# Gadersd/whisper-burn

Hardware: NVIDIA H100
Metric: audio-seconds/sec (higher is better)
Workload: dtype f32 (fp16-exact weights, fp32 activations/accumulate)

## Files before the change

### whisper-burn_b200/csrc/decoder.h

```cpp
#pragma once
#include <stdint.h>

#include "../host/beam_fixed.hpp"
#include "wb_internal.h"

namespace wb {

constexpr int DEC_KC = 8;

struct DecLayer {
    const float *ln1_g, *ln1_b, *ln2_g, *ln2_b, *ln3_g, *ln3_b;
    float ln1_eps, ln2_eps, ln3_eps;
    const void *Wqkv, *Wo, *Wcq, *Wco, *W1, *W2;
    const float *bqkv, *bo, *bcq, *bco, *b1, *b2;
};
enum { D5_KIND_LN = 0, D5_KIND_ATTN, D5_KIND_GEMM };
enum { D5_ST_LN_EMB = 0, D5_ST_LN_FOLD, D5_ST_LN_FOLD_NOPUB, D5_ST_LN_X, D5_ST_PLANES, D5_ST_CROSS };
enum { D5_EM_QKV = 0, D5_EM_RESID, D5_EM_CQ, D5_EM_HID, D5_EM_PART, D5_EM_LOGITS };
struct Dec5Desc {
    int kind = D5_KIND_ATTN;
    const void* W = nullptr;
    const float* bias = nullptr;
    int N = 0, n_slabs = 1, stage = 0, emit = 0;
    const float *g = nullptr, *b = nullptr;
// ... 16 lines not shown
    const void* E_tiled = nullptr;
    const float *lnf_g = nullptr, *lnf_b = nullptr;
    float lnf_eps = 1e-5f;
    float *x = nullptr, *q = nullptr, *att = nullptr, *hid = nullptr;
    float* ypart = nullptr;
    const Dec5Desc* d5 = nullptr;
    void *att_pl = nullptr, *hid_pl = nullptr;
    float* lgbuf = nullptr;
    int lg_slices = 1;
    void *kc = nullptr, *vc = nullptr;
    const void* ckv = nullptr;
    int kv_half = 0;
    int kv_row0 = 0;
    const int* row_window = nullptr;
    const int64_t* win_row_off = nullptr;
    const int* win_T = nullptr;
    const int* anc = nullptr;
    int n_splits = 1;
    float *part_o = nullptr, *part_m = nullptr, *part_l = nullptr;
    int* tokens = nullptr;
    const int* cur_tok = nullptr;
    int use_cur_tok = 0;
    int pos0 = 0, n_steps = 1, logits_from = 0;
    const uint8_t* is_special = nullptr;
    int mask_mode = 0;
    int k = 1, greedy = 0, eot = -1;
    int *lengths = nullptr, *finished = nullptr;
    int *topk_id = nullptr;
    float* topk_lp = nullptr;
    float* logits_out = nullptr;
    float *lg_m = nullptr, *lg_s = nullptr, *lg_v = nullptr;
    int* lg_i = nullptr;
    int *pos = nullptr, *n_unfinished = nullptr, *steps_done = nullptr;
    unsigned int* bar = nullptr;
    const void* d6_pack = nullptr;
    const float* d6_params = nullptr;
    unsigned long long* trace = nullptr;
    int trace_cap = 0;
    int beam = 0, n_win = 0, max_depth = 0;
    int* anc_alt = nullptr;
    int* slot_live = nullptr;
    beamfx::Head* bm_head = nullptr;
    int* bm_seq = nullptr;
    int* bm_cnt = nullptr;
    int* bm_win = nullptr;
    int* bm_out = nullptr;
    int* bm_out_len = nullptr;
};
void launch_dec3(const DecArgs& a, int n_ctas, bool w_half, cudaStream_t st);
bool launch_dec4(const DecArgs& a, bool w_half, cudaStream_t st);
struct Dec6Pack {
    DevBuf<uint8_t> pack;
    DevBuf<float> params;
};
bool launch_dec6(DecArgs a, const Model& m, Dec6Pack& pack, cudaStream_t st);
struct Dec5Tables {
    DevBuf<Dec5Desc> unsplit;
    DevBuf<Dec5Desc> split;
};
void dec5_build_tables(const Model& m, int n_sm, Dec5Tables& t);
int launch_dec5(const DecArgs& a, const Dec5Tables& t, int n_ctas, bool w_half, cudaStream_t st);
size_t dec5_plane_uint4(int d);

void launch_dec_anc_identity(int* anc, int R, int t_max, cudaStream_t st);
void launch_dec_reorder(const int* anc_old, int* anc_new, const int* parent, const int* pos_ptr, int R, int t_max,
                        cudaStream_t st);

}
```

### whisper-burn_b200/csrc/decoder6.cu

```cuda
#include <cooperative_groups.h>

#include <cstdlib>

#include "dec_common.cuh"
#include "wgmma.cuh"

namespace cg = cooperative_groups;

namespace wb {

namespace {

constexpr int NCW = 8;
constexpr int NPROD = 1;
constexpr int W_PROD = NCW;
constexpr int NTH6 = (NCW + NPROD) * 32;
constexpr int SLOT = 16384;
constexpr int NSLOT = 8;
constexpr int LG_NBUF = 2;
constexpr int BX_SLAB = 1024;

template <int D>
struct Geo {
    static constexpr int H = D / 64, CS = H, NS = 4 * D / CS, SEND = D + 4;
    static constexpr int pad128(int n) { return (n + 127) / 128 * 128; }
    static constexpr int OFF_QKV = 0, OFF_O = OFF_QKV + 192 * D * 2, OFF_CQ = OFF_O + D * 64 * 2, OFF_CO = OFF_CQ + 64 * D * 2,
                         OFF_W1 = OFF_CO + D * 64 * 2, OFF_W2 = OFF_W1 + NS * D * 2, PACK = OFF_W2 + D * NS * 2;
    static_assert(D % 128 == 0 && NS % 128 == 0, "only the 192- and 64-row segments end in a 64-row tile");
    static constexpr int P_LN1G = 0, P_LN1B = D, P_LN2G = 2 * D, P_LN2B = 3 * D, P_LN3G = 4 * D, P_LN3B = 5 * D, P_BO = 6 * D,
                         P_BCO = 7 * D, P_B2 = 8 * D, P_BQKV = 9 * D, P_BCQ = 9 * D + 192, P_B1 = 9 * D + 256, P_EPS = 9 * D + 256 + NS, PARAMS = 9 * D + 256 + NS + 4;
    static constexpr int KMAX = D > NS ? D : NS;
    static_assert(PARAMS % 4 == 0 && SEND % 4 == 0 && NS % 64 == 0 && D % 64 == 0, "layout");
};

__device__ __forceinline__ uint32_t s32(const void* p) { return (uint32_t)__cvta_generic_to_shared(p); }
__device__ __forceinline__ void mbar_init(uint64_t* bar, uint32_t count) { asm volatile("mbarrier.init.shared::cta.b64 [%0], %1;" ::"r"(s32(bar)), "r"(count)); }
__device__ __forceinline__ void mbar_expect_tx(uint64_t* bar, uint32_t bytes) {
    asm volatile("mbarrier.arrive.expect_tx.shared::cta.b64 _, [%0], %1;" ::"r"(s32(bar)), "r"(bytes) : "memory");
}
__device__ __forceinline__ void mbar_arrive(uint64_t* bar) { asm volatile("mbarrier.arrive.shared::cta.b64 _, [%0];" ::"r"(s32(bar)) : "memory"); }
__device__ long long g_watchdog = 20000000000LL;
__device__ __forceinline__ void mbar_wait(uint64_t* bar, uint32_t parity) {
    const long long WATCHDOG = g_watchdog;
    const uint32_t b = s32(bar);
    const long long t0 = clock64();
    for (;;) {
        uint32_t done;
        asm volatile("{\n.reg .pred p;\nmbarrier.try_wait.parity.shared::cta.b64 p, [%1], %2;\nselp.u32 %0, 1, 0, p;\n}" : "=r"(done) : "r"(b), "r"(parity) : "memory");
        if (done) return;
        if (clock64() - t0 > WATCHDOG) __trap();
    }
}
__device__ __forceinline__ void bulk_g2s(void* dst, const void* src, uint32_t bytes, uint64_t* bar) {
    asm volatile("cp.async.bulk.shared::cluster.global.mbarrier::complete_tx::bytes [%0], [%1], %2, [%3];" ::"r"(s32(dst)), "l"(src), "r"(bytes), "r"(s32(bar)) : "memory");
}
__device__ __forceinline__ void bulk_s2peer(void* dst_local, const void* src, uint32_t bytes, uint64_t* bar_local, uint32_t rank) {
    uint32_t rd, rb;
    asm volatile("mapa.shared::cluster.u32 %0, %1, %2;" : "=r"(rd) : "r"(s32(dst_local)), "r"(rank));
    asm volatile("mapa.shared::cluster.u32 %0, %1, %2;" : "=r"(rb) : "r"(s32(bar_local)), "r"(rank));
    asm volatile("cp.async.bulk.shared::cluster.shared::cta.mbarrier::complete_tx::bytes [%0], [%1], %2, [%3];" ::"r"(rd), "r"(s32(src)), "r"(bytes), "r"(rb) : "memory");
}
__device__ __forceinline__ void bar_consumers() { asm volatile("bar.sync 1, 256;" ::: "memory"); }
__device__ __forceinline__ void bar_all() { asm volatile("bar.sync 2, %0;" ::"n"(NTH6) : "memory"); }
__device__ __forceinline__ float group8_sum(float v) {
    v += __shfl_xor_sync(0xffffffffu, v, 1);
    v += __shfl_xor_sync(0xffffffffu, v, 2);
    v += __shfl_xor_sync(0xffffffffu, v, 4);
    return v;
}
__device__ __host__ __forceinline__ uint32_t sw128_off(int row, int k, int slab_bytes) {
    return (uint32_t)((k >> 6) * slab_bytes + row * 128 + ((((k & 63) >> 3) ^ (row & 7)) << 4) + (k & 7) * 2);
}

template <typename KVT>
__device__ __forceinline__ int hdim(int l8, int i) {
    if constexpr (sizeof(KVT) == 4) return (i < 4 ? 4 * l8 : 32 + 4 * l8) + (i & 3);
    else return 8 * l8 + i;
}
template <typename KVT>
// ... 159 lines not shown
                }
                o.out[row] = v;
            } else if (o.mode == EM_CQ) {
                o.out[row] = __fmul_rn(__fadd_rn(s, o.bias[row]), o.scale);
            } else {
                o.out[row] = gelu_erf(__fadd_rn(s, o.bias[row]));
            }
        }
    }
    c.tile += (uint32_t)n_tiles;
    c.n += (uint32_t)(n_tiles * n_slabs);
    bar_consumers();
    return c;
}

template <int D>
__device__ __noinline__ void ln6(const float* x_s, const float* g, const float* b, float eps, int eps_outside, uint8_t* bx) {
    const int tid = threadIdx.x, lane = tid & 31;
    float v[D / 32];
    float sum = 0.0f;
#pragma unroll
    for (int i = 0; i < D / 32; ++i) { v[i] = x_s[lane + 32 * i]; sum += v[i]; }
    sum = warp_sum(sum);
    const float mean = __fdiv_rn(sum, (float)D);
    float q = 0.0f;
#pragma unroll
    for (int i = 0; i < D / 32; ++i) { const float dv = __fsub_rn(v[i], mean); q = __fadd_rn(q, __fmul_rn(dv, dv)); }
    q = warp_sum(q);
    const float var = __fdiv_rn(q, (float)D);
    const float den = eps_outside ? __fadd_rn(__fsqrt_rn(var), eps) : __fsqrt_rn(__fadd_rn(var, eps));
#pragma unroll 1
    for (int c = tid; c < D; c += 256) bx_store(bx, c, __fadd_rn(__fmul_rn(__fdiv_rn(__fsub_rn(x_s[c], mean), den), g[c]), b[c]));
}

__device__ __noinline__ void attn_merge6(const float* wm, const float* wl, const float* wo, uint8_t* bx, float* rec) {
    const int tid = threadIdx.x;
    bar_consumers();
    if (tid < 64) {
        float M = -INFINITY;
#pragma unroll
        for (int w2 = 0; w2 < NCW; ++w2) M = fmaxf(M, wm[w2]);
        float Ls = 0.0f, o = 0.0f;
#pragma unroll
        for (int w2 = 0; w2 < NCW; ++w2) {
            const float sc = wm[w2] > -INFINITY ? expf(wm[w2] - M) : 0.0f;
            Ls += sc * wl[w2];
            o += sc * wo[w2 * 64 + tid];
        }
        bx_store(bx, tid, o);
        if (tid == 0) { rec[0] = M; rec[1] = Ls; }
    }
}

enum { MODE_SUM = 0, MODE_ATTN = 1 };

template <int D>
__device__ __noinline__ void combine6(const float* pr, uint64_t* bar, uint32_t parity, int mode, const float* bias, float* x_s, float* wsrc_s) {
    constexpr int CS = Geo<D>::CS, SEND = Geo<D>::SEND;
    const int tid = threadIdx.x;
    if (tid == 0) mbar_expect_tx(bar, CS * SEND * 4);
    mbar_wait(bar, parity);
    if (tid < CS) {
        const float* me = pr + tid * SEND + D;
        wsrc_s[tid] = mode == MODE_SUM ? 1.0f : me[0] > -INFINITY ? __fdiv_rn(1.0f, me[1]) : 0.0f;
    }
    bar_consumers();
#pragma unroll 1
    for (int c = tid; c < D; c += 256) {
        float acc = bias[c];
#pragma unroll 4
        for (int s = 0; s < CS; ++s) acc = fmaf(wsrc_s[s], pr[s * SEND + c], acc);
        x_s[c] = __fadd_rn(x_s[c], acc);
    }
    bar_consumers();
}

template <typename KVT, bool ANC>
__device__ __forceinline__ void self_attn6_body(const float* qkv_s, const KVT* kbase, const KVT* vbase, int ld, int p, const int* anc,
                                                int64_t row_ld, float* wm, float* wl, float* wo) {
    const int warp = threadIdx.x >> 5, lane = threadIdx.x & 31, rg = lane >> 3, l8 = lane & 7;
    float q[8];
#pragma unroll
    for (int i = 0; i < 8; ++i) q[i] = qkv_s[hdim<KVT>(l8, i)];
    Softmax8 A;
    A.init();
    float kf[4][8], vf[4][8];
    const int j0 = warp * 4 + rg;
#pragma unroll
    for (int u = 0; u < 4; ++u) {
        const int j = j0 + 32 * u;
        if (j < p) {
            const int64_t off = ANC ? (int64_t)__ldcg(anc + j) * row_ld + (int64_t)j * ld : (int64_t)j * ld;
            load_row8<KVT>(kbase + off, l8, 0, kf[u], false);
            load_row8<KVT>(vbase + off, l8, 0, vf[u], false);
        } else if (j == p) {
#pragma unroll
            for (int i = 0; i < 8; ++i) { kf[u][i] = qkv_s[64 + hdim<KVT>(l8, i)]; vf[u][i] = qkv_s[128 + hdim<KVT>(l8, i)]; }
        } else {
#pragma unroll
            for (int i = 0; i < 8; ++i) { kf[u][i] = 0.0f; vf[u][i] = 0.0f; }
        }
    }
#pragma unroll
    for (int u = 0; u < 4; ++u) {
        float s = 0.0f;
#pragma unroll
        for (int i = 0; i < 8; ++i) s = fmaf(q[i], kf[u][i], s);
        s = group8_sum(s);
        if (j0 + 32 * u <= p) A.add(s, vf[u]);
    }
    A.merge_xor(8);
    A.merge_xor(16);
    if (rg == 0) {
#pragma unroll
        for (int i = 0; i < 8; ++i) wo[warp * 64 + hdim<KVT>(l8, i)] = A.o[i];
        if (l8 == 0) { wm[warp] = A.m; wl[warp] = A.l; }
    }
}
template <typename KVT>
__device__ __noinline__ void self_attn6(const float* qkv_s, const KVT* kbase, const KVT* vbase, int ld, int p, float* wm, float* wl, float* wo) {
    self_attn6_body<KVT, false>(qkv_s, kbase, vbase, ld, p, nullptr, 0, wm, wl, wo);
}
template <typename KVT>
__device__ __noinline__ void self_attn6_anc(const float* qkv_s, const KVT* kbase, const KVT* vbase, int ld, int p, const int* anc, int64_t row_ld,
                                            float* wm, float* wl, float* wo) {
    self_attn6_body<KVT, true>(qkv_s, kbase, vbase, ld, p, anc, row_ld, wm, wl, wo);
}

__device__ __forceinline__ void cand_insert(float* lv, int* li, float v, int n) {
    if (!(v > lv[DEC_KC - 1] || (v == lv[DEC_KC - 1] && n < li[DEC_KC - 1]))) return;
    int k = DEC_KC - 1;
    for (; k > 0 && (v > lv[k - 1] || (v == lv[k - 1] && n < li[k - 1])); --k) { lv[k] = lv[k - 1]; li[k] = li[k - 1]; }
    lv[k] = v;
    li[k] = n;
}

template <typename KVT>
__device__ __noinline__ uint32_t cross_attn6(const Pipe P, uint32_t n, int* slot_cnt, const float* q2_s, int T, float* wm, float* wl, float* wo) {
    constexpr int ROWB = 128 * (int)sizeof(KVT), KPC = SLOT / ROWB;
    const int warp = threadIdx.x >> 5, lane = threadIdx.x & 31, rg = lane >> 3, l8 = lane & 7;
    float q[8];
#pragma unroll
    for (int i = 0; i < 8; ++i) q[i] = q2_s[hdim<KVT>(l8, i)];
    Softmax8 A;
    A.init();
#pragma unroll 1
    for (int k0 = 0; k0 < T; k0 += KPC) {
        const int nk = min(KPC, T - k0);
        const uint32_t slot = n % NSLOT;
        mbar_wait(P.full + slot, (n / NSLOT) & 1);
        const uint8_t* blk = P.ring + slot * SLOT;
#pragma unroll 2
        for (int kk = warp * 4 + rg; kk < nk; kk += 32) {
            const int par = (k0 + kk) & 1;
            const KVT* rowp = reinterpret_cast<const KVT*>(blk + (size_t)kk * ROWB);
            float kf[8], vf[8];
            load_row8<KVT>(rowp, l8, par, kf, true);
            load_row8<KVT>(rowp + 64, l8, par, vf, true);
            float s = 0.0f;
#pragma unroll
            for (int i = 0; i < 8; ++i) s = fmaf(q[i], kf[i], s);
            const unsigned int gm = 0xffu << (lane & 24);
            s += __shfl_xor_sync(gm, s, 1);
            s += __shfl_xor_sync(gm, s, 2);
            s += __shfl_xor_sync(gm, s, 4);
            A.add(s, vf);
        }
        __syncwarp();
        if (lane == 0 && atomicAdd(slot_cnt + slot, 1) == NCW - 1) {
            slot_cnt[slot] = 0;
            mbar_arrive(P.empty + slot);
        }
        ++n;
    }
    __syncwarp();
    A.merge_xor(8);
    A.merge_xor(16);
    if (rg == 0) {
#pragma unroll
        for (int i = 0; i < 8; ++i) wo[warp * 64 + hdim<KVT>(l8, i)] = A.o[i];
        if (l8 == 0) { wm[warp] = A.m; wl[warp] = A.l; }
    }
    return n;
}

constexpr int BM_LIVE = 24;
constexpr int BM_NX = 3 * BM_LIVE + 3 * NCW * beamfx::MAX_NODES;
__device__ __noinline__ void finish_beam(const DecArgs& a, int p, int depth, const int* anc_cur, uint8_t* scratch, const int* live, int* nx,
                                         int* ctl) {
    namespace fx = beamfx;
    const int tid = threadIdx.x, warp = tid >> 5, lane = tid & 31;
    const int R = a.R, B = a.beam, t_max = a.t_max, NW = a.n_win;
    int* nx_par = nx;
    int* nx_tok = nx_par + BM_LIVE;
    int* nx_live = nx_tok + BM_LIVE;
    int* pk_src = nx_live + BM_LIVE + warp * 3 * fx::MAX_NODES;
    int* pk_tok = pk_src + fx::MAX_NODES;
    int* pk_len = pk_tok + fx::MAX_NODES;
    constexpr int RINGW = NSLOT * SLOT / NCW;
    static_assert(160 * DEC_KC * 8 <= RINGW, "finisher candidate scratch");
    for (int r = warp; r < R; r += NCW) {
        if (!live[r]) continue;
        const int NP = gridDim.x;
        float rm[5], rs[5];
#pragma unroll
        for (int k = 0; k < 5; ++k) {
            const int c = min(lane + 32 * k, NP - 1);
// ... 108 lines not shown
            const int s = pk_src[i], tk = pk_tok[i], ln = pk_len[i] - (tk >= 0 ? 1 : 0);
            for (int j = lane; j < ln; j += 32) dst[i * t_max + j] = __ldcg(src + s * t_max + j);
            if (lane == 0 && tk >= 0) dst[i * t_max + ln] = tk;
        }
        __syncwarp();
    }
    bar_consumers();
    if (tid == 0) {
        int open = 0;
        for (int w = 0; w < NW; ++w) open += __ldcg(a.bm_win + 2 * w + 1) ? 0 : 1;
        ctl[2] = (depth + 1 >= a.max_depth || open == 0) ? 1 : 0;
        ctl[3] = open;
    }
    bar_consumers();
    if (ctl[2] == 0) {
        int* an = (depth & 1) ? const_cast<int*>(a.anc) : a.anc_alt;
        if (tid < R) {
            a.slot_live[tid] = nx_live[tid];
            if (nx_live[tid]) a.tokens[(int64_t)tid * t_max + p + 1] = nx_tok[tid];
        }
        const int P = p + 2;
        for (int q = tid; q < R * P; q += 256) {
            const int r = q / P, j = q % P;
            if (nx_live[r]) an[(int64_t)r * t_max + j] = j <= p ? __ldcg(anc_cur + (int64_t)nx_par[r] * t_max + j) : r;
        }
    } else {
        for (int w = warp; w < NW; w += NCW) {
            const int buf = __ldcg(a.bm_win + 2 * w);
            const fx::Head* hs = a.bm_head + ((size_t)buf * NW + w) * fx::MAX_NODES;
            int best = 0, len = 0;
            if (lane == 0) {
                const int n = __ldcg(a.bm_cnt + buf * NW + w);
                fx::Head hn[fx::MAX_NODES];
                for (int b = 0; b < n; ++b) { hn[b].log_prob = __ldcg(&hs[b].log_prob); hn[b].finished = __ldcg(&hs[b].finished); }
                best = max(fx::max_by_last(hn, n), 0);
                len = n > 0 ? __ldcg(&hs[best].len) : 0;
                a.bm_out_len[w] = len;
            }
            best = __shfl_sync(0xffffffffu, best, 0);
            len = __shfl_sync(0xffffffffu, len, 0);
            const int* s = a.bm_seq + (((size_t)buf * NW + w) * fx::MAX_NODES + best) * t_max;
            for (int j = lane; j < len; j += 32) a.bm_out[(int64_t)w * t_max + j] = __ldcg(s + j);
        }
        if (tid == 0) {
            *a.steps_done = depth + 1;
            *a.pos = p + 1;
            *a.n_unfinished = ctl[3];
            a.bar[3] = 1;
        }
    }
    bar_consumers();
}

template <int D, int NT8, typename KVT, bool BEAM = false>
__global__ void __launch_bounds__(NTH6, 1)
dec6_kernel(const DecArgs a) {
    using G = Geo<D>;
    constexpr int CS = G::CS, NS = G::NS, SEND = G::SEND, PARAMS = G::PARAMS;
    constexpr int KPC = SLOT / (128 * (int)sizeof(KVT));
    constexpr int ROWB = 128 * (int)sizeof(KVT);
    extern __shared__ __align__(1024) unsigned char smraw_[];
    uint8_t* smraw = reinterpret_cast<uint8_t*>((reinterpret_cast<uintptr_t>(smraw_) + 1023) & ~(uintptr_t)1023);
    cg::cluster_group cl = cg::this_cluster();
    const int tid = threadIdx.x, warp = tid >> 5, lane = tid & 31;
    const int rank = (int)cl.block_rank(), h = rank;
    const int cluster_id = blockIdx.x / CS, n_clusters = gridDim.x / CS;
    const int L = a.L, V = a.V, R = a.R, t_max = a.t_max;

    uint8_t* ring_mem = smraw;
    uint8_t* bx = ring_mem + NSLOT * SLOT;
    float* params = reinterpret_cast<float*>(bx + (G::KMAX / 64) * BX_SLAB);
    float* part = params + 2 * PARAMS;
    float* y_s = part + 2 * CS * SEND;
    float* x_s = y_s + 2 * SEND;
    float* qkv_s = x_s + D;
    float* q2_s = qkv_s + 192;
    float* hid_s = q2_s + 64;
    float* wsrc_s = hid_s + NS;
    float* wm = wsrc_s + 16;
    float* wl = wm + 8;
    float* wo = wl + 8;
    int* ctl = reinterpret_cast<int*>(wo + 512);
    int* slot_cnt = ctl + 4;
    uint64_t* bars = reinterpret_cast<uint64_t*>(slot_cnt + NSLOT);
    uint64_t* full = bars;
    uint64_t* empty = full + NSLOT;
    uint64_t* pfull = empty + NSLOT;
    uint64_t* pfree = pfull + 2;
    uint64_t* pbar = pfree + 2;
    uint64_t* lg_bar = pbar + 2;
    int* live_s = reinterpret_cast<int*>(lg_bar + NCW * LG_NBUF);
    int* live_rows = live_s + 2 * BM_LIVE;
    int* n_live_s = live_rows + 2 * BM_LIVE;
    int* nx_s = n_live_s + 2;
    uint4* pl_hi = reinterpret_cast<uint4*>(params);
    uint4* pl_lo = pl_hi + NT8 * (D / 32) * 32;
    float* red = reinterpret_cast<float*>(pl_lo + NT8 * (D / 32) * 32);

    if (tid == 0) {
        for (int i = 0; i < NSLOT; ++i) { mbar_init(full + i, 1); mbar_init(empty + i, 1); slot_cnt[i] = 0; }
        for (int i = 0; i < 2; ++i) { mbar_init(pfull + i, 1); mbar_init(pfree + i, NCW); mbar_init(pbar + i, 1); }
        for (int i = 0; i < NCW * LG_NBUF; ++i) mbar_init(lg_bar + i, 1);
        ctl[0] = 0; ctl[1] = 0;
        asm volatile("fence.mbarrier_init.release.cluster;" ::: "memory");
    }
    for (int i = tid; i < (G::KMAX / 64) * BX_SLAB / 16; i += NTH6) reinterpret_cast<uint4*>(bx)[i] = make_uint4(0, 0, 0, 0);
    auto snapshot_live = [&](int buf) {
        if (tid < R) live_s[buf * BM_LIVE + tid] = __ldcg(a.slot_live + tid);
        bar_consumers();
        if (tid == 0) {
            int n = 0;
            for (int r = 0; r < R; ++r)
                if (live_s[buf * BM_LIVE + r]) live_rows[buf * BM_LIVE + n++] = r;
            n_live_s[buf] = n;
        }
    };
    if constexpr (BEAM) {
        if (tid < 256) snapshot_live(0);
    }
    cl.sync();
    Pipe P;
    P.ring = ring_mem; P.full = full; P.empty = empty; P.bx = bx;

    const uint8_t* pack = reinterpret_cast<const uint8_t*>(a.d6_pack);
    const float* gparams = a.d6_params;
    constexpr int S_D = D / 64, S_NS = NS / 64;

    if (warp >= W_PROD) {
        const uint32_t pw = (uint32_t)(warp - W_PROD);
        uint32_t n = 0, pl = 0;
        auto push = [&](const void* src, uint32_t bytes) {
            if (n % NPROD == pw) {
                const uint32_t slot = n % NSLOT;
                if (n >= NSLOT) mbar_wait(empty + slot, ((n / NSLOT) - 1) & 1);
                mbar_expect_tx(full + slot, bytes);
                bulk_g2s(ring_mem + slot * SLOT, src, bytes, full + slot);
            }
            ++n;
        };
        for (int step = 0; step < a.n_steps; ++step) {
            if (lane == 0) {
                const int n_iter = BEAM ? n_live_s[step & 1] : R;
                for (int it = cluster_id; it < n_iter; it += n_clusters) {
                    const int row = BEAM ? live_rows[(step & 1) * BM_LIVE + it] : it;
                    const int w = __ldg(a.row_window + row);
                    const int T = __ldg(a.win_T + w);
                    for (int l = 0; l < L; ++l) {
                        if (pw == 0) {
                            const uint32_t b = pl & 1, u = pl >> 1;
                            if (u >= 1) mbar_wait(pfree + b, (u - 1) & 1);
                            mbar_expect_tx(pfull + b, PARAMS * 4);
                            bulk_g2s(params + b * PARAMS, gparams + ((size_t)l * CS + rank) * PARAMS, PARAMS * 4, pfull + b);
                        }
                        ++pl;
                        const uint8_t* base = pack + ((size_t)l * CS + rank) * G::PACK;
                        auto seg = [&](int off, int N, int K) {
                            const uint8_t* src = base + off;
                            for (int r0 = 0; r0 < N; r0 += 128) {
                                const uint32_t bytes = (uint32_t)min(128, N - r0) * 128;
                                for (int sl = 0; sl < K / 64; ++sl, src += bytes) push(src, bytes);
                            }
                        };
                        seg(G::OFF_QKV, 192, D);
                        seg(G::OFF_O, D, 64);
                        seg(G::OFF_CQ, 64, D);
                        {
                            const KVT* kv = reinterpret_cast<const KVT*>(a.ckv) + (size_t)l * a.Mcap * 2 * D + __ldg(a.win_row_off + w) * (int64_t)(2 * D) +
                                            (int64_t)h * T * 128;
                            for (int k0 = 0; k0 < T; k0 += KPC) push(kv + (int64_t)k0 * 128, (uint32_t)(min(KPC, T - k0) * ROWB));
                        }
                        seg(G::OFF_CO, D, 64);
                        seg(G::OFF_W1, NS, D);
                        seg(G::OFF_W2, D, NS);
                    }
                }
            }
            __syncwarp();
            bar_all();
            if (*reinterpret_cast<volatile int*>(ctl) != 0) break;
        }
    } else {
        Counters c{0, 0};
        uint32_t pl = 0;
        uint32_t ph = 0;
        unsigned int gen = 0;
        unsigned int lg_count = 0;
        int tr_n = 0;
        const float scale = a.qk_scale;
        const int gw = blockIdx.x * NCW + warp, n_gw = gridDim.x * NCW;

        auto trace = [&]() {
            if (a.trace && blockIdx.x == 0 && tid == 0 && tr_n < a.trace_cap / 2) a.trace[tr_n++] = gtime();
        };
        auto send = [&]() {
            asm volatile("fence.proxy.async.shared::cta;" ::: "memory");
            bar_consumers();
            if (tid < CS) {
                const uint32_t b = ph & 1;
                bulk_s2peer(part + (b * CS + rank) * SEND, y_s + b * SEND, SEND * 4, pbar + b, (uint32_t)tid);
            }
        };
        auto combine = [&](int mode, const float* bias) {
            combine6<D>(part + (ph & 1) * CS * SEND, pbar + (ph & 1), (ph >> 1) & 1, mode, bias, x_s, wsrc_s);
            ++ph;
        };

#pragma unroll 1
        for (int step = 0; step < a.n_steps; ++step) {
            const int p = a.pos0 + step;
            const bool want_logits = p >= a.logits_from;
            const int depth = p - a.logits_from;
            const int n_iter = BEAM ? n_live_s[step & 1] : R;
            const int* anc_cur = depth > 0 && (depth & 1) ? a.anc_alt : a.anc;
#pragma unroll 1
            for (int it = cluster_id; it < n_iter; it += n_clusters) {
                const int row = BEAM ? live_rows[(step & 1) * BM_LIVE + it] : it;
                {
                    const int tok = __ldcg(a.tokens + (int64_t)row * t_max + p);
                    for (int c2 = tid; c2 < D; c2 += 256) x_s[c2] = __fadd_rn(__ldg(a.tok_emb + (int64_t)tok * D + c2), __ldg(a.pos_emb + (int64_t)p * D + c2));
                }
                const int w = __ldg(a.row_window + row);
                const int T = __ldg(a.win_T + w);
                bar_consumers();
                trace();
#pragma unroll 1
                for (int l = 0; l < L; ++l) {
                    KVT* kcl = reinterpret_cast<KVT*>(a.kc) + (size_t)l * a.Rmax * t_max * D;
                    KVT* vcl = reinterpret_cast<KVT*>(a.vc) + (size_t)l * a.Rmax * t_max * D;
                    if (l > 0) {
                        combine(MODE_SUM, params + ((pl + 1) & 1) * PARAMS + G::P_B2);
                        __syncwarp();
                        if (lane == 0) mbar_arrive(pfree + ((pl + 1) & 1));
                    }
                    trace();
                    mbar_wait(pfull + (pl & 1), (pl >> 1) & 1);
                    const float* prm = params + (pl & 1) * PARAMS;
                    ++pl;
                    float* ys = y_s + (ph & 1) * SEND;
                    ln6<D>(x_s, prm + G::P_LN1G, prm + G::P_LN1B, prm[G::P_EPS + 0], a.eps_outside, bx);
                    KVT* kd = kcl + ((int64_t)row * t_max + p) * D + h * 64;
                    KVT* vd = vcl + ((int64_t)row * t_max + p) * D + h * 64;
                    c = gemv_epi6<KVT>(P, c, 192, S_D, GemvOut<KVT>{EM_QKV, prm + G::P_BQKV, scale, qkv_s, kd, vd});
                    trace();
                    if constexpr (BEAM)
                        self_attn6_anc<KVT>(qkv_s, kcl + h * 64, vcl + h * 64, D, p, anc_cur + (int64_t)row * t_max, (int64_t)t_max * D, wm, wl, wo);
                    else
                        self_attn6<KVT>(qkv_s, kcl + (int64_t)row * t_max * D + h * 64, vcl + (int64_t)row * t_max * D + h * 64, D, p, wm, wl, wo);
                    attn_merge6(wm, wl, wo, bx, ys + D);
                    trace();
                    c = gemv_epi6<KVT>(P, c, D, 1, GemvOut<KVT>{EM_PLAIN, nullptr, 1.0f, ys, nullptr, nullptr});
                    trace();
                    send();
                    trace();
                    combine(MODE_ATTN, prm + G::P_BO);
                    trace();
                    ys = y_s + (ph & 1) * SEND;
                    ln6<D>(x_s, prm + G::P_LN2G, prm + G::P_LN2B, prm[G::P_EPS + 1], a.eps_outside, bx);
                    c = gemv_epi6<KVT>(P, c, 64, S_D, GemvOut<KVT>{EM_CQ, prm + G::P_BCQ, scale, q2_s, nullptr, nullptr});
                    trace();
                    c.n = cross_attn6<KVT>(P, c.n, slot_cnt, q2_s, T, wm, wl, wo);
                    attn_merge6(wm, wl, wo, bx, ys + D);
                    trace();
                    c = gemv_epi6<KVT>(P, c, D, 1, GemvOut<KVT>{EM_PLAIN, nullptr, 1.0f, ys, nullptr, nullptr});
                    trace();
                    send();
                    trace();
                    combine(MODE_ATTN, prm + G::P_BCO);
                    trace();
                    ys = y_s + (ph & 1) * SEND;
                    ln6<D>(x_s, prm + G::P_LN3G, prm + G::P_LN3B, prm[G::P_EPS + 2], a.eps_outside, bx);
                    c = gemv_epi6<KVT>(P, c, NS, S_D, GemvOut<KVT>{EM_HID, prm + G::P_B1, 1.0f, hid_s, nullptr, nullptr});
                    for (int c2 = tid; c2 < NS; c2 += 256) bx_store(bx, c2, hid_s[c2]);
                    trace();
                    c = gemv_epi6<KVT>(P, c, D, S_NS, GemvOut<KVT>{EM_PLAIN, nullptr, 1.0f, ys, nullptr, nullptr});
                    trace();
                    send();
                    trace();
                }
                combine(MODE_SUM, params + ((pl + 1) & 1) * PARAMS + G::P_B2);
                __syncwarp();
                if (lane == 0) mbar_arrive(pfree + ((pl + 1) & 1));
                if (want_logits && rank == 0)
                    for (int c = tid; c < D; c += 256) a.x[(int64_t)row * D + c] = x_s[c];
                bar_consumers();
            }
            int stop = 0;
            if (want_logits) {
                const int lg_g = lane >> 2, lg_t = lane & 3;
                constexpr int KH = D / 2, NCH = KH / 32;
                constexpr uint32_t BLKB = 16 * KH * 2;
                constexpr int RINGW = NSLOT * SLOT / NCW;
                static_assert(LG_NBUF * (int)BLKB <= RINGW, "logits ring");
                const __half* Et = reinterpret_cast<const __half*>(a.E_tiled);
                const int v_tiles = (V + 15) / 16;
                const int R_act = BEAM ? n_live_s[step & 1] : R;
                const bool idle_cta = cluster_id >= R_act;
                const int n_idle_w = max(0, n_clusters - R_act) * CS * NCW;
                const int na = (n_idle_w > 0 && 2 * n_idle_w <= v_tiles) ? 1 : 0;
                const int tiles_a = na * n_idle_w, tiles_b = v_tiles - tiles_a;
                const int iw = ((cluster_id - R_act) * CS + rank) * NCW + warp;
                const int my_a = idle_cta ? na : 0;
                const int my_tiles = my_a + (gw < tiles_b ? (tiles_b - gw + n_gw - 1) / n_gw : 0);
                const int total = my_tiles * 2;
                auto tile_of = [&](int i) { return i < my_a ? iw + i * n_idle_w : tiles_a + gw + (i - my_a) * n_gw; };
                uint8_t* wring = ring_mem + (size_t)warp * RINGW;
                uint64_t* wbar = lg_bar + warp * LG_NBUF;
                auto issue = [&](int it) {
                    if (it < total && lane == 0) {
                        const int vt = tile_of(it >> 1);
                        const int slot = (int)((lg_count + (unsigned int)it) % LG_NBUF);
                        mbar_expect_tx(wbar + slot, BLKB);
                        bulk_g2s(wring + (size_t)slot * BLKB, Et + ((int64_t)vt * 2 + (it & 1)) * 16 * KH, BLKB, wbar + slot);
                    }
                };
                if (idle_cta) {
                    asm volatile("fence.proxy.async.shared::cta;" ::: "memory");
#pragma unroll
                    for (int j = 0; j < LG_NBUF; ++j) issue(j);
                }
                trace();
// ... 271 lines not shown
                        if (lane == 0) {
                            a.topk_id[r] = bii == INT_MAX ? -1 : bii;
                            a.topk_lp[r] = __fsub_rn(__fsub_rn(bvv, mx), lse);
                            if (!__ldcg(a.finished + r)) {
                                a.tokens[(int64_t)r * t_max + p + 1] = bii;
                                a.lengths[r] = p + 2;
                                if (bii == a.eot) a.finished[r] = 1;
                            }
                        }
                    }
                    bar_consumers();
                    if (tid == 0) {
                        __threadfence();
                        asm volatile("st.release.gpu.global.u32 [%0], %1;" ::"l"(a.bar + 2), "r"(gen) : "memory");
                    }
                }
                if (tid == 0) {
                    const long long t0 = clock64(), wd = g_watchdog;
                    while (ld_acquire(a.bar + 2) < gen)
                        if (clock64() - t0 > wd) __trap();
                }
                bar_consumers();
                trace();
                if constexpr (BEAM) {
                    stop = __ldcg(a.bar + 3) != 0;
                } else {
                    int live = 0;
                    for (int r = 0; r < R; ++r) live += __ldcg(a.finished + r) ? 0 : 1;
                    if (live == 0) {
                        stop = 1;
                        if (blockIdx.x == 0 && tid == 0) { *a.pos = p + 1; *a.n_unfinished = 0; *a.steps_done = step + 1; }
                    }
                }
            }
            if constexpr (BEAM) {
                if (!stop) snapshot_live((step + 1) & 1);
            }
            if (tid == 0) ctl[0] = stop;
            asm volatile("fence.proxy.async.shared::cta;" ::: "memory");
            bar_all();
            if (stop) break;
            if (!BEAM && step + 1 == a.n_steps && blockIdx.x == 0 && tid == 0) {
                *a.pos = a.pos0 + a.n_steps;
                int live = 0;
                for (int r = 0; r < R; ++r) live += __ldcg(a.finished + r) ? 0 : 1;
                *a.n_unfinished = live;
                *a.steps_done = a.n_steps;
            }
        }
    }
    cl.sync();
}

template <int D, int NT8, bool BEAM = false>
constexpr size_t dec6_smem() {
    using G = Geo<D>;
    return 1024 + (size_t)NSLOT * SLOT + (size_t)(G::KMAX / 64) * BX_SLAB +
           sizeof(float) * ((size_t)2 * G::PARAMS + 2 * G::CS * G::SEND + 2 * G::SEND + D + 192 + 64 + G::NS + 16 + 8 + 8 + 512 + 4 + NSLOT) +
           8 * (size_t)(2 * NSLOT + 6 + NCW * LG_NBUF) + 64 + (BEAM ? sizeof(int) * (4 * BM_LIVE + 2 + BM_NX) : 0);
}

template <int D, int NT8, typename KVT, bool BEAM = false>
bool launch6_t(const DecArgs& a, cudaStream_t st) {
    using G = Geo<D>;
    static_assert((size_t)2 * NT8 * (D / 32) * 32 * 16 + (size_t)NCW * 8 * NT8 * 16 <= sizeof(float) * (2 * G::PARAMS + 2 * G::CS * G::SEND), "logits scratch must fit the aliased buffers");
    const void* k = (const void*)dec6_kernel<D, NT8, KVT, BEAM>;
    const size_t smem = dec6_smem<D, NT8, BEAM>();
    static ClusterLaunch cl;
    const int n_cl = cl.capacity(k, G::CS, NTH6, smem, "dec6");
    if (n_cl < 1) return false;
    static PerDeviceConfig wd;
    wd.ensure(1, [] {
        if (const char* e = getenv("WB200_WATCHDOG_MS")) {
            const long long ms = atoll(e);
            const long long cyc = ms <= 0 ? (1LL << 62) : ms * 2000000LL;
            WB_CUDA(cudaMemcpyToSymbol(g_watchdog, &cyc, sizeof(cyc)));
        }
        return true;
    });
    void* args[] = {(void*)&a};
    cl.launch(k, G::CS, n_cl, NTH6, smem, args, st, "dec6");
    return true;
}

template <int D>
void build_pack_t(const Model& m, Dec6Pack& pk, cudaStream_t st) {
    using G = Geo<D>;
    const int L = m.dims.n_text_layer;
    pk.pack.alloc((size_t)L * G::CS * G::PACK);
    pk.params.alloc((size_t)L * G::CS * G::PARAMS);
    std::vector<PackSeg> ps;
    std::vector<ParamSeg> qs;
    std::vector<float> eps_h((size_t)L * 4, 0.0f);
    for (int l = 0; l < L; ++l) {
        const DecBlockW& B = m.dec[(size_t)l];
        eps_h[(size_t)l * 4] = B.attn_ln.eps; eps_h[(size_t)l * 4 + 1] = B.cross_ln.eps; eps_h[(size_t)l * 4 + 2] = B.mlp_ln.eps;
    }
    DevBuf<float> eps_d;
    eps_d.alloc(eps_h.size());
    WB_CUDA(cudaMemcpyAsync(eps_d.p, eps_h.data(), eps_h.size() * sizeof(float), cudaMemcpyHostToDevice, st));
    for (int l = 0; l < L; ++l) {
        const DecBlockW& B = m.dec[(size_t)l];
        for (int h = 0; h < G::CS; ++h) {
            const int64_t base = ((int64_t)l * G::CS + h) * G::PACK;
            const int64_t pb = ((int64_t)l * G::CS + h) * G::PARAMS;
            ps.push_back(PackSeg{B.qkv.w16, D, h * 64, 0, 192, D, 64, D, base + G::OFF_QKV});
            ps.push_back(PackSeg{B.out.w16, D, 0, h * 64, D, 64, D, 0, base + G::OFF_O});
            ps.push_back(PackSeg{B.cq.w16, D, h * 64, 0, 64, D, 64, 0, base + G::OFF_CQ});
            ps.push_back(PackSeg{B.cout.w16, D, 0, h * 64, D, 64, D, 0, base + G::OFF_CO});
            ps.push_back(PackSeg{B.mlp1.w16, D, h * G::NS, 0, G::NS, D, G::NS, 0, base + G::OFF_W1});
            ps.push_back(PackSeg{B.mlp2.w16, 4 * D, 0, h * G::NS, D, G::NS, D, 0, base + G::OFF_W2});
            qs.push_back(ParamSeg{B.attn_ln.g, D, pb + G::P_LN1G}); qs.push_back(ParamSeg{B.attn_ln.b, D, pb + G::P_LN1B});
            qs.push_back(ParamSeg{B.cross_ln.g, D, pb + G::P_LN2G}); qs.push_back(ParamSeg{B.cross_ln.b, D, pb + G::P_LN2B});
            qs.push_back(ParamSeg{B.mlp_ln.g, D, pb + G::P_LN3G}); qs.push_back(ParamSeg{B.mlp_ln.b, D, pb + G::P_LN3B});
            qs.push_back(ParamSeg{B.out.b, D, pb + G::P_BO}); qs.push_back(ParamSeg{B.cout.b, D, pb + G::P_BCO}); qs.push_back(ParamSeg{B.mlp2.b, D, pb + G::P_B2});
            for (int part = 0; part < 3; ++part) qs.push_back(ParamSeg{B.qkv.b + part * D + h * 64, 64, pb + G::P_BQKV + part * 64});
            qs.push_back(ParamSeg{B.cq.b + h * 64, 64, pb + G::P_BCQ});
            qs.push_back(ParamSeg{B.mlp1.b + h * G::NS, G::NS, pb + G::P_B1});
            qs.push_back(ParamSeg{eps_d.p + (size_t)l * 4, 4, pb + G::P_EPS});
        }
    }
    DevBuf<PackSeg> dps;
    DevBuf<ParamSeg> dqs;
    dps.alloc(ps.size());
    dqs.alloc(qs.size());
    WB_CUDA(cudaMemcpyAsync(dps.p, ps.data(), ps.size() * sizeof(PackSeg), cudaMemcpyHostToDevice, st));
    WB_CUDA(cudaMemcpyAsync(dqs.p, qs.data(), qs.size() * sizeof(ParamSeg), cudaMemcpyHostToDevice, st));
    dec6_pack_kernel<<<dim3(32, (unsigned)std::min<size_t>(ps.size(), 1024)), 256, 0, st>>>(dps.p, (int)ps.size(), pk.pack.p);
    WB_LAUNCH_CHECK();
    dec6_param_kernel<<<(unsigned)std::min<size_t>(qs.size(), 2048), 128, 0, st>>>(dqs.p, (int)qs.size(), pk.params.p);
    WB_LAUNCH_CHECK();
    WB_CUDA(cudaStreamSynchronize(st));
}

}

bool launch_dec6(DecArgs a, const Model& m, Dec6Pack& pk, cudaStream_t st) {
    const bool beam = a.beam > 1;
    if (!m.fp16_exact || a.R > BM_LIVE || a.R < 1 || a.use_cur_tok || a.logits_out != nullptr) return false;
    if (!beam && (a.k != 1 || !a.greedy || a.anc != nullptr)) return false;
    if (beam && (a.beam > beamfx::MAX_BEAM || a.k != a.beam || a.greedy || a.R != a.n_win * a.beam || a.pos0 != 0 || a.max_depth < 1 ||
                 a.anc == nullptr || a.anc_alt == nullptr || a.slot_live == nullptr || a.bm_head == nullptr)) return false;
    if ((a.d != 128 && a.d != 384) || a.H * 64 != a.d || a.E_tiled == nullptr || a.t_max > 128) return false;
    if (pk.pack.p == nullptr) {
        if (a.d == 384) build_pack_t<384>(m, pk, st);
        else build_pack_t<128>(m, pk, st);
    }
    a.d6_pack = pk.pack.p;
    a.d6_params = pk.params.p;
#define WB_D6(DD, NT8_)                                                                                                  \
    (beam ? (a.kv_half ? launch6_t<DD, NT8_, __half, true>(a, st) : launch6_t<DD, NT8_, float, true>(a, st))             \
          : (a.kv_half ? launch6_t<DD, NT8_, __half>(a, st) : launch6_t<DD, NT8_, float>(a, st)))
    if (a.d == 384) return a.R <= 8 ? WB_D6(384, 1) : WB_D6(384, 3);
    return a.R <= 8 ? WB_D6(128, 1) : WB_D6(128, 3);
#undef WB_D6
}

}
```

Before: 2485.

## Split each head across two CTAs in dec6 for small greedy batches

Adds a PAIR variant of the dec6 cluster kernel that uses 2*H CTAs per cluster when R is small and decoding is greedy. Each head's work is shared by two CTAs: cross-attention KV is split in halves and merged with a softmax-rescaled combine, the output projection is split by columns, and MLP slabs are halved. A separate pair-specific weight pack is built. The aim is to spread the per-row decoder work over more SMs when there are few rows, at the cost of larger clusters, extra partial-sum exchange and extra pack memory.

```diff
diff --git a/whisper-burn_b200/csrc/decoder.h b/whisper-burn_b200/csrc/decoder.h
--- a/whisper-burn_b200/csrc/decoder.h
+++ b/whisper-burn_b200/csrc/decoder.h
@@ -92,6 +92,8 @@
 struct Dec6Pack {
     DevBuf<uint8_t> pack;
     DevBuf<float> params;
+    DevBuf<uint8_t> pair_pack;
+    DevBuf<float> pair_params;
 };
 bool launch_dec6(DecArgs a, const Model& m, Dec6Pack& pack, cudaStream_t st);
 struct Dec5Tables {
diff --git a/whisper-burn_b200/csrc/decoder6.cu b/whisper-burn_b200/csrc/decoder6.cu
--- a/whisper-burn_b200/csrc/decoder6.cu
+++ b/whisper-burn_b200/csrc/decoder6.cu
@@ -19,12 +19,14 @@
 constexpr int NSLOT = 8;
 constexpr int LG_NBUF = 2;
 constexpr int BX_SLAB = 1024;
-
-template <int D>
+constexpr int DEC6_PAIR_ROWS = 8;
+
+template <int D, bool PAIR = false>
 struct Geo {
-    static constexpr int H = D / 64, CS = H, NS = 4 * D / CS, SEND = D + 4;
+    static constexpr int H = D / 64, CS = PAIR ? 2 * H : H, NS = 4 * D / CS, SEND = D + 4;
+    static constexpr int NO = PAIR ? D / 2 : D;
     static constexpr int pad128(int n) { return (n + 127) / 128 * 128; }
-    static constexpr int OFF_QKV = 0, OFF_O = OFF_QKV + 192 * D * 2, OFF_CQ = OFF_O + D * 64 * 2, OFF_CO = OFF_CQ + 64 * D * 2,
+    static constexpr int OFF_QKV = 0, OFF_O = OFF_QKV + 192 * D * 2, OFF_CQ = OFF_O + NO * 64 * 2, OFF_CO = OFF_CQ + 64 * D * 2,
                          OFF_W1 = OFF_CO + D * 64 * 2, OFF_W2 = OFF_W1 + NS * D * 2, PACK = OFF_W2 + D * NS * 2;
     static_assert(D % 128 == 0 && NS % 128 == 0, "only the 192- and 64-row segments end in a 64-row tile");
     static constexpr int P_LN1G = 0, P_LN1B = D, P_LN2G = 2 * D, P_LN2B = 3 * D, P_LN3G = 4 * D, P_LN3B = 5 * D, P_BO = 6 * D,
@@ -290,17 +292,25 @@
     }
 }
 
-enum { MODE_SUM = 0, MODE_ATTN = 1 };
-
-template <int D>
+enum { MODE_SUM = 0, MODE_ATTN = 1, MODE_PAIR = 2 };
+
+template <int D, bool PAIR>
 __device__ __noinline__ void combine6(const float* pr, uint64_t* bar, uint32_t parity, int mode, const float* bias, float* x_s, float* wsrc_s) {
-    constexpr int CS = Geo<D>::CS, SEND = Geo<D>::SEND;
+    constexpr int CS = Geo<D, PAIR>::CS, SEND = Geo<D, PAIR>::SEND;
     const int tid = threadIdx.x;
     if (tid == 0) mbar_expect_tx(bar, CS * SEND * 4);
     mbar_wait(bar, parity);
     if (tid < CS) {
         const float* me = pr + tid * SEND + D;
-        wsrc_s[tid] = mode == MODE_SUM ? 1.0f : me[0] > -INFINITY ? __fdiv_rn(1.0f, me[1]) : 0.0f;
+        if (PAIR && mode == MODE_PAIR) {
+            const float* r0 = pr + (tid & ~1) * SEND + D;
+            const float* r1 = r0 + SEND;
+            const float M = fmaxf(r0[0], r1[0]);
+            const float den = (r0[0] > -INFINITY ? expf(r0[0] - M) * r0[1] : 0.0f) + (r1[0] > -INFINITY ? expf(r1[0] - M) * r1[1] : 0.0f);
+            wsrc_s[tid] = me[0] > -INFINITY ? __fdiv_rn(expf(me[0] - M), den) : 0.0f;
+        } else {
+            wsrc_s[tid] = mode == MODE_SUM ? 1.0f : me[0] > -INFINITY ? __fdiv_rn(1.0f, me[1]) : 0.0f;
+        }
     }
     bar_consumers();
 #pragma unroll 1
@@ -374,7 +384,7 @@
 }
 
 template <typename KVT>
-__device__ __noinline__ uint32_t cross_attn6(const Pipe P, uint32_t n, int* slot_cnt, const float* q2_s, int T, float* wm, float* wl, float* wo) {
+__device__ __noinline__ uint32_t cross_attn6(const Pipe P, uint32_t n, int* slot_cnt, const float* q2_s, int kb, int T, float* wm, float* wl, float* wo) {
     constexpr int ROWB = 128 * (int)sizeof(KVT), KPC = SLOT / ROWB;
     const int warp = threadIdx.x >> 5, lane = threadIdx.x & 31, rg = lane >> 3, l8 = lane & 7;
     float q[8];
@@ -390,7 +400,7 @@
         const uint8_t* blk = P.ring + slot * SLOT;
 #pragma unroll 2
         for (int kk = warp * 4 + rg; kk < nk; kk += 32) {
-            const int par = (k0 + kk) & 1;
+            const int par = (kb + k0 + kk) & 1;
             const KVT* rowp = reinterpret_cast<const KVT*>(blk + (size_t)kk * ROWB);
             float kf[8], vf[8];
             load_row8<KVT>(rowp, l8, par, kf, true);
@@ -605,18 +615,21 @@
     bar_consumers();
 }
 
-template <int D, int NT8, typename KVT, bool BEAM = false>
+template <int D, int NT8, typename KVT, bool BEAM = false, bool PAIR = false>
 __global__ void __launch_bounds__(NTH6, 1)
 dec6_kernel(const DecArgs a) {
-    using G = Geo<D>;
-    constexpr int CS = G::CS, NS = G::NS, SEND = G::SEND, PARAMS = G::PARAMS;
+    static_assert(!(BEAM && PAIR), "the beam mode runs on the H-CTA shape");
+    using G = Geo<D, PAIR>;
+    constexpr int CS = G::CS, NS = G::NS, SEND = G::SEND, PARAMS = G::PARAMS, NO = G::NO;
     constexpr int KPC = SLOT / (128 * (int)sizeof(KVT));
     constexpr int ROWB = 128 * (int)sizeof(KVT);
     extern __shared__ __align__(1024) unsigned char smraw_[];
     uint8_t* smraw = reinterpret_cast<uint8_t*>((reinterpret_cast<uintptr_t>(smraw_) + 1023) & ~(uintptr_t)1023);
     cg::cluster_group cl = cg::this_cluster();
     const int tid = threadIdx.x, warp = tid >> 5, lane = tid & 31;
-    const int rank = (int)cl.block_rank(), h = rank;
+    const int rank = (int)cl.block_rank(), h = PAIR ? rank >> 1 : rank, half = PAIR ? rank & 1 : 0;
+    auto kv_begin = [&](int T) { return half * ((T + 1) >> 1); };
+    auto kv_count = [&](int T) { return PAIR ? (half ? T >> 1 : (T + 1) >> 1) : T; };
     const int cluster_id = blockIdx.x / CS, n_clusters = gridDim.x / CS;
     const int L = a.L, V = a.V, R = a.R, t_max = a.t_max;
 
@@ -715,12 +728,13 @@
                             }
                         };
                         seg(G::OFF_QKV, 192, D);
-                        seg(G::OFF_O, D, 64);
+                        seg(G::OFF_O, NO, 64);
                         seg(G::OFF_CQ, 64, D);
                         {
+                            const int nk = kv_count(T);
                             const KVT* kv = reinterpret_cast<const KVT*>(a.ckv) + (size_t)l * a.Mcap * 2 * D + __ldg(a.win_row_off + w) * (int64_t)(2 * D) +
-                                            (int64_t)h * T * 128;
-                            for (int k0 = 0; k0 < T; k0 += KPC) push(kv + (int64_t)k0 * 128, (uint32_t)(min(KPC, T - k0) * ROWB));
+                                            ((int64_t)h * T + kv_begin(T)) * 128;
+                            for (int k0 = 0; k0 < nk; k0 += KPC) push(kv + (int64_t)k0 * 128, (uint32_t)(min(KPC, nk - k0) * ROWB));
                         }
                         seg(G::OFF_CO, D, 64);
                         seg(G::OFF_W1, NS, D);
@@ -754,7 +768,7 @@
             }
         };
         auto combine = [&](int mode, const float* bias) {
-            combine6<D>(part + (ph & 1) * CS * SEND, pbar + (ph & 1), (ph >> 1) & 1, mode, bias, x_s, wsrc_s);
+            combine6<D, PAIR>(part + (ph & 1) * CS * SEND, pbar + (ph & 1), (ph >> 1) & 1, mode, bias, x_s, wsrc_s);
             ++ph;
         };
 
@@ -800,8 +814,10 @@
                     else
                         self_attn6<KVT>(qkv_s, kcl + (int64_t)row * t_max * D + h * 64, vcl + (int64_t)row * t_max * D + h * 64, D, p, wm, wl, wo);
                     attn_merge6(wm, wl, wo, bx, ys + D);
-                    trace();
-                    c = gemv_epi6<KVT>(P, c, D, 1, GemvOut<KVT>{EM_PLAIN, nullptr, 1.0f, ys, nullptr, nullptr});
+                    if constexpr (PAIR)
+                        for (int c2 = tid; c2 < NO; c2 += 256) ys[(half ^ 1) * NO + c2] = 0.0f;
+                    trace();
+                    c = gemv_epi6<KVT>(P, c, NO, 1, GemvOut<KVT>{EM_PLAIN, nullptr, 1.0f, ys + half * NO, nullptr, nullptr});
                     trace();
                     send();
                     trace();
@@ -811,14 +827,14 @@
                     ln6<D>(x_s, prm + G::P_LN2G, prm + G::P_LN2B, prm[G::P_EPS + 1], a.eps_outside, bx);
                     c = gemv_epi6<KVT>(P, c, 64, S_D, GemvOut<KVT>{EM_CQ, prm + G::P_BCQ, scale, q2_s, nullptr, nullptr});
                     trace();
-                    c.n = cross_attn6<KVT>(P, c.n, slot_cnt, q2_s, T, wm, wl, wo);
+                    c.n = cross_attn6<KVT>(P, c.n, slot_cnt, q2_s, kv_begin(T), kv_count(T), wm, wl, wo);
                     attn_merge6(wm, wl, wo, bx, ys + D);
                     trace();
                     c = gemv_epi6<KVT>(P, c, D, 1, GemvOut<KVT>{EM_PLAIN, nullptr, 1.0f, ys, nullptr, nullptr});
                     trace();
                     send();
                     trace();
-                    combine(MODE_ATTN, prm + G::P_BCO);
+                    combine(PAIR ? MODE_PAIR : MODE_ATTN, prm + G::P_BCO);
                     trace();
                     ys = y_s + (ph & 1) * SEND;
                     ln6<D>(x_s, prm + G::P_LN3G, prm + G::P_LN3B, prm[G::P_EPS + 2], a.eps_outside, bx);
@@ -1196,23 +1212,23 @@
     cl.sync();
 }
 
-template <int D, int NT8, bool BEAM = false>
+template <int D, int NT8, bool BEAM = false, bool PAIR = false>
 constexpr size_t dec6_smem() {
-    using G = Geo<D>;
+    using G = Geo<D, PAIR>;
     return 1024 + (size_t)NSLOT * SLOT + (size_t)(G::KMAX / 64) * BX_SLAB +
            sizeof(float) * ((size_t)2 * G::PARAMS + 2 * G::CS * G::SEND + 2 * G::SEND + D + 192 + 64 + G::NS + 16 + 8 + 8 + 512 + 4 + NSLOT) +
            8 * (size_t)(2 * NSLOT + 6 + NCW * LG_NBUF) + 64 + (BEAM ? sizeof(int) * (4 * BM_LIVE + 2 + BM_NX) : 0);
 }
 
-template <int D, int NT8, typename KVT, bool BEAM = false>
+template <int D, int NT8, typename KVT, bool BEAM = false, bool PAIR = false>
 bool launch6_t(const DecArgs& a, cudaStream_t st) {
-    using G = Geo<D>;
+    using G = Geo<D, PAIR>;
     static_assert((size_t)2 * NT8 * (D / 32) * 32 * 16 + (size_t)NCW * 8 * NT8 * 16 <= sizeof(float) * (2 * G::PARAMS + 2 * G::CS * G::SEND), "logits scratch must fit the aliased buffers");
-    const void* k = (const void*)dec6_kernel<D, NT8, KVT, BEAM>;
-    const size_t smem = dec6_smem<D, NT8, BEAM>();
+    const void* k = (const void*)dec6_kernel<D, NT8, KVT, BEAM, PAIR>;
+    const size_t smem = dec6_smem<D, NT8, BEAM, PAIR>();
     static ClusterLaunch cl;
-    const int n_cl = cl.capacity(k, G::CS, NTH6, smem, "dec6");
-    if (n_cl < 1) return false;
+    const int n_cl = cl.capacity(k, G::CS, NTH6, smem, PAIR ? "dec6 pair" : "dec6");
+    if (n_cl < (PAIR ? a.R : 1)) return false;
     static PerDeviceConfig wd;
     wd.ensure(1, [] {
         if (const char* e = getenv("WB200_WATCHDOG_MS")) {
@@ -1223,16 +1239,16 @@
         return true;
     });
     void* args[] = {(void*)&a};
-    cl.launch(k, G::CS, n_cl, NTH6, smem, args, st, "dec6");
+    cl.launch(k, G::CS, n_cl, NTH6, smem, args, st, PAIR ? "dec6 pair" : "dec6");
     return true;
 }
 
-template <int D>
-void build_pack_t(const Model& m, Dec6Pack& pk, cudaStream_t st) {
-    using G = Geo<D>;
+template <int D, bool PAIR>
+void build_pack_t(const Model& m, DevBuf<uint8_t>& pack, DevBuf<float>& params, cudaStream_t st) {
+    using G = Geo<D, PAIR>;
     const int L = m.dims.n_text_layer;
-    pk.pack.alloc((size_t)L * G::CS * G::PACK);
-    pk.params.alloc((size_t)L * G::CS * G::PARAMS);
+    pack.alloc((size_t)L * G::CS * G::PACK);
+    params.alloc((size_t)L * G::CS * G::PARAMS);
     std::vector<PackSeg> ps;
     std::vector<ParamSeg> qs;
     std::vector<float> eps_h((size_t)L * 4, 0.0f);
@@ -1245,22 +1261,23 @@
     WB_CUDA(cudaMemcpyAsync(eps_d.p, eps_h.data(), eps_h.size() * sizeof(float), cudaMemcpyHostToDevice, st));
     for (int l = 0; l < L; ++l) {
         const DecBlockW& B = m.dec[(size_t)l];
-        for (int h = 0; h < G::CS; ++h) {
-            const int64_t base = ((int64_t)l * G::CS + h) * G::PACK;
-            const int64_t pb = ((int64_t)l * G::CS + h) * G::PARAMS;
+        for (int r = 0; r < G::CS; ++r) {
+            const int h = PAIR ? r >> 1 : r, s = PAIR ? r & 1 : 0;
+            const int64_t base = ((int64_t)l * G::CS + r) * G::PACK;
+            const int64_t pb = ((int64_t)l * G::CS + r) * G::PARAMS;
             ps.push_back(PackSeg{B.qkv.w16, D, h * 64, 0, 192, D, 64, D, base + G::OFF_QKV});
-            ps.push_back(PackSeg{B.out.w16, D, 0, h * 64, D, 64, D, 0, base + G::OFF_O});
+            ps.push_back(PackSeg{B.out.w16, D, s * G::NO, h * 64, G::NO, 64, G::NO, 0, base + G::OFF_O});
             ps.push_back(PackSeg{B.cq.w16, D, h * 64, 0, 64, D, 64, 0, base + G::OFF_CQ});
             ps.push_back(PackSeg{B.cout.w16, D, 0, h * 64, D, 64, D, 0, base + G::OFF_CO});
-            ps.push_back(PackSeg{B.mlp1.w16, D, h * G::NS, 0, G::NS, D, G::NS, 0, base + G::OFF_W1});
-            ps.push_back(PackSeg{B.mlp2.w16, 4 * D, 0, h * G::NS, D, G::NS, D, 0, base + G::OFF_W2});
+            ps.push_back(PackSeg{B.mlp1.w16, D, r * G::NS, 0, G::NS, D, G::NS, 0, base + G::OFF_W1});
+            ps.push_back(PackSeg{B.mlp2.w16, 4 * D, 0, r * G::NS, D, G::NS, D, 0, base + G::OFF_W2});
             qs.push_back(ParamSeg{B.attn_ln.g, D, pb + G::P_LN1G}); qs.push_back(ParamSeg{B.attn_ln.b, D, pb + G::P_LN1B});
             qs.push_back(ParamSeg{B.cross_ln.g, D, pb + G::P_LN2G}); qs.push_back(ParamSeg{B.cross_ln.b, D, pb + G::P_LN2B});
             qs.push_back(ParamSeg{B.mlp_ln.g, D, pb + G::P_LN3G}); qs.push_back(ParamSeg{B.mlp_ln.b, D, pb + G::P_LN3B});
             qs.push_back(ParamSeg{B.out.b, D, pb + G::P_BO}); qs.push_back(ParamSeg{B.cout.b, D, pb + G::P_BCO}); qs.push_back(ParamSeg{B.mlp2.b, D, pb + G::P_B2});
             for (int part = 0; part < 3; ++part) qs.push_back(ParamSeg{B.qkv.b + part * D + h * 64, 64, pb + G::P_BQKV + part * 64});
             qs.push_back(ParamSeg{B.cq.b + h * 64, 64, pb + G::P_BCQ});
-            qs.push_back(ParamSeg{B.mlp1.b + h * G::NS, G::NS, pb + G::P_B1});
+            qs.push_back(ParamSeg{B.mlp1.b + r * G::NS, G::NS, pb + G::P_B1});
             qs.push_back(ParamSeg{eps_d.p + (size_t)l * 4, 4, pb + G::P_EPS});
         }
     }
@@ -1270,9 +1287,9 @@
     dqs.alloc(qs.size());
     WB_CUDA(cudaMemcpyAsync(dps.p, ps.data(), ps.size() * sizeof(PackSeg), cudaMemcpyHostToDevice, st));
     WB_CUDA(cudaMemcpyAsync(dqs.p, qs.data(), qs.size() * sizeof(ParamSeg), cudaMemcpyHostToDevice, st));
-    dec6_pack_kernel<<<dim3(32, (unsigned)std::min<size_t>(ps.size(), 1024)), 256, 0, st>>>(dps.p, (int)ps.size(), pk.pack.p);
+    dec6_pack_kernel<<<dim3(32, (unsigned)std::min<size_t>(ps.size(), 1024)), 256, 0, st>>>(dps.p, (int)ps.size(), pack.p);
     WB_LAUNCH_CHECK();
-    dec6_param_kernel<<<(unsigned)std::min<size_t>(qs.size(), 2048), 128, 0, st>>>(dqs.p, (int)qs.size(), pk.params.p);
+    dec6_param_kernel<<<(unsigned)std::min<size_t>(qs.size(), 2048), 128, 0, st>>>(dqs.p, (int)qs.size(), params.p);
     WB_LAUNCH_CHECK();
     WB_CUDA(cudaStreamSynchronize(st));
 }
@@ -1286,9 +1303,21 @@
     if (beam && (a.beam > beamfx::MAX_BEAM || a.k != a.beam || a.greedy || a.R != a.n_win * a.beam || a.pos0 != 0 || a.max_depth < 1 ||
                  a.anc == nullptr || a.anc_alt == nullptr || a.slot_live == nullptr || a.bm_head == nullptr)) return false;
     if ((a.d != 128 && a.d != 384) || a.H * 64 != a.d || a.E_tiled == nullptr || a.t_max > 128) return false;
+    if (!beam && a.R <= DEC6_PAIR_ROWS) {
+        if (pk.pair_pack.p == nullptr) {
+            if (a.d == 384) build_pack_t<384, true>(m, pk.pair_pack, pk.pair_params, st);
+            else build_pack_t<128, true>(m, pk.pair_pack, pk.pair_params, st);
+        }
+        DecArgs ap = a;
+        ap.d6_pack = pk.pair_pack.p;
+        ap.d6_params = pk.pair_params.p;
+        const bool ran = a.d == 384 ? (a.kv_half ? launch6_t<384, 1, __half, false, true>(ap, st) : launch6_t<384, 1, float, false, true>(ap, st))
+                                    : (a.kv_half ? launch6_t<128, 1, __half, false, true>(ap, st) : launch6_t<128, 1, float, false, true>(ap, st));
+        if (ran) return true;
+    }
     if (pk.pack.p == nullptr) {
-        if (a.d == 384) build_pack_t<384>(m, pk, st);
-        else build_pack_t<128>(m, pk, st);
+        if (a.d == 384) build_pack_t<384, false>(m, pk.pack, pk.params, st);
+        else build_pack_t<128, false>(m, pk.pack, pk.params, st);
     }
     a.d6_pack = pk.pack.p;
     a.d6_params = pk.params.p;
```

New measurement: 2463 (median of 6 runs). No clear change (-0.9%).
